# YannDubs/disentangling-vae

Hardware: AMD Instinct MI355X
Metric: images/sec (whole node) at 64x64x3, btcvae loss (higher is better)
Workload: dtype f32; 1 GPU; btcvae_celeba (BASELINE.json configs[3]): Burgess VAE 64x64x3, btcvae loss, z=10, tensor handed to _train_iteration B=1024 global (1024 per GPU), Adam lr 0.0005, n_data=202599, fwd+loss+bwd+Adam; batch_per_gpu=1024, global_batch=1024, parallelism=dp1

## Files before the change

disentangling-vae_amd/csrc/conv_up_thin_mm.hip:

```cpp
#include "recon_epilogue.h"

namespace dvae {

#define UTM_ROWS 12
#define UTM_COLS 34
#define UTM_TILE (UTM_ROWS * UTM_COLS * 32)
#define UTM_BR 11
#define UTM_NPOS (UTM_BR * 33)
#define UTM_OR 22
#define UTM_STAGE (3 * UTM_OR * 64)

__device__ __forceinline__ float sigmoid_hw_mm(float v) { return sigmoid_aten(v); }

#ifndef UTM_VARIANT
#define UTM_VARIANT 13
#endif
#ifndef UTM_ABL
#define UTM_ABL 0
#endif
__device__ __forceinline__ void utm_barrier() {
  if (UTM_VARIANT & 4) { wait_lgkmcnt0(); barrier_nofence(); }
  else __syncthreads();
}

template <bool FUSE, int DIST, typename TT>
__global__ __launch_bounds__(512, 4) void k_up_thin_mm(const float* __restrict__ small, const float* __restrict__ wimg,
                                                       const float* __restrict__ bias, float* __restrict__ out, int N,
                                                       int n_units, const TT* __restrict__ target, float* __restrict__ g,
                                                       const float* __restrict__ coef, float* __restrict__ partials) {
  extern __shared__ __attribute__((aligned(16))) float smem[];
  float* tin = smem;
  float* stage = smem + UTM_TILE;
  float* redl = stage + UTM_STAGE;
  float* wl = redl + 8;
  const int tid = threadIdx.x, lane = tid & 63;
  const int wv = __builtin_amdgcn_readfirstlane(tid >> 6);
  const int j = lane & 15, kg = lane >> 4;
  const float gs = FUSE ? coef[DVAE_C_INV_B] : 0.f;
  float lsum = 0.f;

  for (int e = tid; e < UTM_TILE / 4; e += 512) reinterpret_cast<f32x4*>(tin)[e] = f32x4{0.f, 0.f, 0.f, 0.f};

  for (int e = tid; e < 32 * 64 / 4; e += 512) reinterpret_cast<f32x4*>(wl)[e] = reinterpret_cast<const f32x4*>(wimg)[e];
  const float bv = (kg < 3 && bias) ? bias[kg] : 0.f;

  int xb[3], soff[3];
  int key0[3];
  bool x0ok[3], x1ok[3];
#pragma unroll
  for (int s = 0; s < 3; ++s) {
    const int pos0 = 16 * (3 * wv + s) + j;
    const bool pvalid = pos0 < UTM_NPOS;
    const int pos = pvalid ? pos0 : UTM_NPOS - 1;
    const int rq = pos / 33, cq = pos - 33 * rq;
    xb[s] = (rq * UTM_COLS + cq) * 32;
    key0[s] = cq & 7;
    soff[s] = (kg * UTM_OR + 2 * rq) * 64 + 2 * cq - 1;
    x0ok[s] = pvalid && kg < 3 && cq > 0;
    x1ok[s] = pvalid && kg < 3 && cq < 32;
  }
  const bool tile3 = 16 * (3 * wv + 2) < UTM_NPOS;
  const int within = tid & 255, rhalf = tid >> 8;
  const int pgo = rhalf * 1024 + within * 4;
  const int ci_ld = (within >> 3) + 1;
  const int plo = (rhalf * UTM_COLS + ci_ld) * 32 + (((within & 7) ^ (ci_ld & 7)) << 2);
  int bso[3], bgo[3], brow[3];
#pragma unroll
  for (int k = 0; k < 3; ++k) {
    const int e = tid + 512 * k;
    const int c = e / (UTM_OR * 16), rem = e - c * (UTM_OR * 16), r = rem >> 4, x4 = rem & 15;
    brow[k] = e < 3 * UTM_OR * 16 ? r : -1000;
    bso[k] = (c * UTM_OR + r) * 64 + 4 * x4;
    bgo[k] = (c * 64 + r) * 64 + 4 * x4;
  }
  __syncthreads();

  f32x4 pf[6];
  auto load_tile = [&](int unit) {
    const int n = unit / 3, u3 = unit - 3 * n;
    const int sy0 = UTM_BR * u3 - 1;
    const float* base = small + ((long)n * 32 + sy0) * 1024 + pgo;
#pragma unroll
    for (int k = 0; k < 6; ++k) {
      const int sy = sy0 + 2 * k + rhalf;
      pf[k] = f32x4{0.f, 0.f, 0.f, 0.f};
      if (sy >= 0 && sy < 32 && !((UTM_ABL & 16) && N > 0)) pf[k] = *reinterpret_cast<const f32x4*>(base + 2048 * k);
    }
  };
  if ((int)blockIdx.x < n_units) load_tile(blockIdx.x);
  for (int unit = blockIdx.x; unit < n_units; unit += gridDim.x) {
    const int n = unit / 3, u3 = unit - 3 * n;
    const int Y0 = UTM_OR * u3 - 1;
    const long img0 = ((long)n * 3 * 64 + Y0) * 64;
    f32x4 tg[3];
    uchar4 tg8[3];
    auto load_targets_k = [&](int k) {
      const int Y = Y0 + brow[k];
      tg[k] = f32x4{0.f, 0.f, 0.f, 0.f};
      tg8[k] = make_uchar4(0, 0, 0, 0);
      if (Y >= 0 && Y < 64) {
        if constexpr (sizeof(TT) == 4) tg[k] = *reinterpret_cast<const f32x4*>(target + img0 + bgo[k]);
        else tg8[k] = *reinterpret_cast<const uchar4*>(target + img0 + bgo[k]);
      }
    };
    auto load_targets = [&]() {
#pragma unroll
      for (int k = 0; k < 3; ++k) {
        const int Y = Y0 + brow[k];
        tg[k] = f32x4{0.f, 0.f, 0.f, 0.f};
        tg8[k] = make_uchar4(0, 0, 0, 0);
        if (Y >= 0 && Y < 64 && !((UTM_ABL & 4) && N > 0)) {
          if constexpr (sizeof(TT) == 4) tg[k] = *reinterpret_cast<const f32x4*>(target + img0 + bgo[k]);
          else tg8[k] = *reinterpret_cast<const uchar4*>(target + img0 + bgo[k]);
        }
      }
    };
#pragma unroll
    for (int k = 0; k < 6; ++k) *reinterpret_cast<f32x4*>(tin + plo + 2 * UTM_COLS * 32 * k) = pf[k];
    if ((UTM_VARIANT & 1) && unit + (int)gridDim.x < n_units) load_tile(unit + gridDim.x);
    if (FUSE && (UTM_VARIANT & 2)) load_targets();
    if (FUSE && (UTM_VARIANT & 16)) load_targets_k(0);
    utm_barrier();
    f32x4 acc[3];
#pragma unroll
    for (int s = 0; s < 3; ++s) acc[s] = f32x4{0.f, 0.f, 0.f, 0.f};
#pragma unroll
    for (int tap = 0; tap < 4; ++tap) {
      const int a = tap >> 1, b = tap & 1;
      f32x4 x[3][2];
      float wr[8];
#pragma unroll
      for (int i = 0; i < 8; ++i) wr[i] = wl[(tap * 8 + i) * 64 + lane];
#pragma unroll
      for (int s = 0; s < 3; ++s) {
        if (s == 2 && !tile3) continue;
        const int key = (key0[s] + b) & 7;
        const float* px = tin + xb[s] + (a * UTM_COLS + b) * 32;
        x[s][0] = *reinterpret_cast<const f32x4*>(px + (((2 * kg) ^ key) << 2));
        x[s][1] = *reinterpret_cast<const f32x4*>(px + (((2 * kg + 1) ^ key) << 2));
      }
#pragma unroll
      for (int i = 0; i < 8; ++i) {
#pragma unroll
        for (int s = 0; s < 3; ++s) {
          if (s == 2 && !tile3) continue;
          if (!((UTM_ABL & 1) && N > 0)) acc[s] = __builtin_amdgcn_mfma_f32_16x16x4f32(wr[i], x[s][i >> 2][i & 3], acc[s], 0, 0, 0);
        }
      }
    }
    if (FUSE && (UTM_VARIANT & 8)) load_targets();
    if (FUSE && (UTM_VARIANT & 16)) { load_targets_k(1); load_targets_k(2); }
#pragma unroll
    for (int s = 0; s < 3; ++s) {
      if (s == 2 && !tile3) continue;
      float* sp = stage + soff[s];
      if (x0ok[s]) { sp[0] = acc[s][0] + bv; sp[64] = acc[s][2] + bv; }
      if (x1ok[s]) { sp[1] = acc[s][1] + bv; sp[65] = acc[s][3] + bv; }
    }
    utm_barrier();
    if (!(UTM_VARIANT & 1) && unit + (int)gridDim.x < n_units) load_tile(unit + gridDim.x);
    if (FUSE && !(UTM_VARIANT & (2 | 8 | 16))) load_targets();
    if (FUSE && sizeof(TT) != 4) {
#pragma unroll
      for (int k = 0; k < 3; ++k) tg[k] = f32x4{to_unit(tg8[k].x), to_unit(tg8[k].y), to_unit(tg8[k].z), to_unit(tg8[k].w)};
    }
#pragma unroll
    for (int k = 0; k < 3; ++k) {
      const int Y = Y0 + brow[k];
      if (Y < 0 || Y >= 64) continue;
      f32x4 v = *reinterpret_cast<const f32x4*>(stage + bso[k]);
      f32x4 gl = {0.f, 0.f, 0.f, 0.f};
#pragma unroll
      for (int q = 0; q < 4; ++q) {
        if ((UTM_ABL & 2) && N > 0) {
          gl[q] = v[q] + tg[k][q];
        } else if (FUSE && DIST == DVAE_REC_BERNOULLI) {
          float y, glq;
          lsum += sigmoid_bce_logit(v[q], tg[k][q], &y, &glq);
          v[q] = y;
          gl[q] = gs * glq;
        } else {
          const float y = sigmoid_hw_mm(v[q]);
          v[q] = y;
          if (FUSE) {
            float glq, gr;
            lsum += recon_elem(y, tg[k][q], DIST, &glq, &gr);
            gl[q] = gs * glq;
          }
        }
      }
      if ((UTM_ABL & 8) && N > 0) { lsum += v[0] + v[1] + v[2] + v[3] + gl[0] + gl[1] + gl[2] + gl[3]; continue; }
      *reinterpret_cast<f32x4*>(out + img0 + bgo[k]) = v;
      if (FUSE) *reinterpret_cast<f32x4*>(g + img0 + bgo[k]) = gl;
    }
  }
  if (FUSE) {
    const float v = wave_sum(lsum);
    __syncthreads();
    if (lane == 0) redl[wv] = v;
    __syncthreads();
    if (tid == 0) {
      float s = 0.f;
#pragma unroll
      for (int w = 0; w < 8; ++w) s += redl[w];
      partials[blockIdx.x] = s;
    }
    for (int k = gridDim.x + blockIdx.x * 512 + tid; k < DVAE_REC_NPART; k += gridDim.x * 512) partials[k] = 0.f;
  }
}

int launch_up_thin_mm(const float* small, const float* wimg, const float* bias, const void* target, int target_u8, float* out,
                      float* g, int dist, const float* coef, float* partials, int N, int act, hipStream_t s) {
  static const bool off = env_off("DVAE_UP_THIN_MM");
  static const int min_n = env_int("DVAE_UP_THIN_MM_MIN_N", 1);
  if (off || N < min_n || act != DVAE_ACT_SIGMOID) return 1;
  if ((((uintptr_t)small | (uintptr_t)out | (uintptr_t)g) & 15) != 0 || ((uintptr_t)target & (target_u8 ? 3 : 15)) != 0) return 1;
  const int n_units = 3 * N;
  static const int cap = env_int("DVAE_UP_THIN_MM_GRID", 512);
  const int grid = n_units < cap ? n_units : cap;
  constexpr size_t lds = (size_t)(UTM_TILE + UTM_STAGE + 8 + 32 * 64) * sizeof(float);
#define UTM_GO(FUSE_, DIST_, TT_)                                                                                         \
  do {                                                                                                                    \
    static DeviceOnce attr;                                                                                               \
    if (attr.first())                                                                                                     \
      (void)hipFuncSetAttribute((const void*)k_up_thin_mm<FUSE_, DIST_, TT_>, hipFuncAttributeMaxDynamicSharedMemorySize, (int)lds); \
    hipLaunchKernelGGL((k_up_thin_mm<FUSE_, DIST_, TT_>), dim3(grid), dim3(512), lds, s, small, wimg, bias, out, N, n_units,      \
                       (const TT_*)target, g, coef, partials);                                                           \
  } while (0)
  if (!target) UTM_GO(false, 0, float);
  else if (target_u8) {
    if (dist == DVAE_REC_BERNOULLI) UTM_GO(true, DVAE_REC_BERNOULLI, uint8_t);
    else if (dist == DVAE_REC_GAUSSIAN) UTM_GO(true, DVAE_REC_GAUSSIAN, uint8_t);
    else UTM_GO(true, DVAE_REC_LAPLACE, uint8_t);
  } else {
    if (dist == DVAE_REC_BERNOULLI) UTM_GO(true, DVAE_REC_BERNOULLI, float);
    else if (dist == DVAE_REC_GAUSSIAN) UTM_GO(true, DVAE_REC_GAUSSIAN, float);
    else UTM_GO(true, DVAE_REC_LAPLACE, float);
  }
#undef UTM_GO
  DVAE_CHECK_LAUNCH();
  return 0;
}

}
```

Measured before the change: 991,200 images/s.

## Stream input tiles into LDS via direct global-to-LDS DMA from dedicated waves

Replaces the register-staged prefetch of the input tile (global load into registers, then LDS store) with direct global-to-LDS DMA transfers issued by the last UTM_NDW waves. The next tile is issued after the epilogue barrier and awaited with vmcnt-based waits before the compute barrier. Boundary rows are now zeroed explicitly instead of loading zeros. The third target/epilogue slot is restricted to wave 0, and the variant default changes to match the new schedule. This cuts VGPR pressure and LDS write instructions, but depends on correct vmcnt accounting and explicit zeroing of halo rows.

```diff
diff --git a/disentangling-vae_amd/csrc/conv_up_thin_mm.hip b/disentangling-vae_amd/csrc/conv_up_thin_mm.hip
--- a/disentangling-vae_amd/csrc/conv_up_thin_mm.hip
+++ b/disentangling-vae_amd/csrc/conv_up_thin_mm.hip
@@ -13,11 +13,15 @@
 __device__ __forceinline__ float sigmoid_hw_mm(float v) { return sigmoid_aten(v); }
 
 #ifndef UTM_VARIANT
-#define UTM_VARIANT 13
+#define UTM_VARIANT 12
 #endif
 #ifndef UTM_ABL
 #define UTM_ABL 0
 #endif
+#ifndef UTM_NDW
+#define UTM_NDW 2
+#endif
+static_assert(UTM_NDW == 1 || UTM_NDW == 2 || UTM_NDW == 4, "a wave's transfers stay inside one tile row; wave 0 never issues");
 __device__ __forceinline__ void utm_barrier() {
   if (UTM_VARIANT & 4) { wait_lgkmcnt0(); barrier_nofence(); }
   else __syncthreads();
@@ -42,10 +46,10 @@
   for (int e = tid; e < UTM_TILE / 4; e += 512) reinterpret_cast<f32x4*>(tin)[e] = f32x4{0.f, 0.f, 0.f, 0.f};
 
   for (int e = tid; e < 32 * 64 / 4; e += 512) reinterpret_cast<f32x4*>(wl)[e] = reinterpret_cast<const f32x4*>(wimg)[e];
-  const float bv = (kg < 3 && bias) ? bias[kg] : 0.f;
-
-  int xb[3], soff[3];
-  int key0[3];
+  float bv = (kg < 3 && bias) ? bias[kg] : 0.f;
+  asm volatile("" : "+v"(bv));
+
+  int xb[3], soff[3], key0[3];
   bool x0ok[3], x1ok[3];
 #pragma unroll
   for (int s = 0; s < 3; ++s) {
@@ -60,10 +64,9 @@
     x1ok[s] = pvalid && kg < 3 && cq < 32;
   }
   const bool tile3 = 16 * (3 * wv + 2) < UTM_NPOS;
-  const int within = tid & 255, rhalf = tid >> 8;
-  const int pgo = rhalf * 1024 + within * 4;
-  const int ci_ld = (within >> 3) + 1;
-  const int plo = (rhalf * UTM_COLS + ci_ld) * 32 + (((within & 7) ^ (ci_ld & 7)) << 2);
+  const bool dmaw = wv >= 8 - UTM_NDW, k2on = wv == 0;
+  const unsigned dvoff = (unsigned)(((lane >> 3) << 7) + (((lane & 7) ^ (((lane >> 3) + 1) & 7)) << 4));
+  const unsigned lds_tin = (unsigned)(unsigned long long)(__attribute__((address_space(3))) void*)tin;
   int bso[3], bgo[3], brow[3];
 #pragma unroll
   for (int k = 0; k < 3; ++k) {
@@ -75,30 +78,28 @@
   }
   __syncthreads();
 
-  f32x4 pf[6];
-  auto load_tile = [&](int unit) {
+  constexpr int UTM_NST = (UTM_ABL & 8) ? 0 : (FUSE ? 4 : 2);
+  constexpr int UTM_NTG = !FUSE ? 0 : (UTM_VARIANT & 2) ? ((UTM_ABL & 4) ? 0 : 2) : (UTM_VARIANT & 16) ? 1 : 0;
+  auto issue_tile = [&](int unit) {
     const int n = unit / 3, u3 = unit - 3 * n;
-    const int sy0 = UTM_BR * u3 - 1;
-    const float* base = small + ((long)n * 32 + sy0) * 1024 + pgo;
-#pragma unroll
-    for (int k = 0; k < 6; ++k) {
-      const int sy = sy0 + 2 * k + rhalf;
-      pf[k] = f32x4{0.f, 0.f, 0.f, 0.f};
-      if (sy >= 0 && sy < 32 && !((UTM_ABL & 16) && N > 0)) pf[k] = *reinterpret_cast<const f32x4*>(base + 2048 * k);
+    const float* row0 = small + ((long)n * 32 + UTM_BR * u3) * 1024 + (wv - (8 - UTM_NDW)) * 256;
+#pragma unroll
+    for (int k = 0; k < 4 * UTM_ROWS / UTM_NDW; ++k) {
+      const int ri = (UTM_NDW * k) >> 2, t = (UTM_NDW * k) & 3;
+      if ((ri == 0 && u3 == 0) || (ri == UTM_ROWS - 1 && u3 == 2) || ((UTM_ABL & 16) && N > 0)) continue;
+      const unsigned dst = lds_tin + (unsigned)((ri * UTM_COLS + 8 * t + 1) * 128) + (unsigned)(wv - (8 - UTM_NDW)) * 1024u;
+      lds_dma16_masked(row0 + (ri - 1) * 1024 + t * 256, dvoff, __builtin_amdgcn_readfirstlane(dst), ~0ull);
     }
   };
-  if ((int)blockIdx.x < n_units) load_tile(blockIdx.x);
+  if (dmaw) issue_tile(blockIdx.x);
   for (int unit = blockIdx.x; unit < n_units; unit += gridDim.x) {
-    const int n = unit / 3, u3 = unit - 3 * n;
-    const int Y0 = UTM_OR * u3 - 1;
+    const int n = unit / 3, u3 = unit - 3 * n, Y0 = UTM_OR * u3 - 1;
     const long img0 = ((long)n * 3 * 64 + Y0) * 64;
-    f32x4 tg[3];
-    uchar4 tg8[3];
+    f32x4 tg[3]; uchar4 tg8[3];
     auto load_targets_k = [&](int k) {
       const int Y = Y0 + brow[k];
-      tg[k] = f32x4{0.f, 0.f, 0.f, 0.f};
-      tg8[k] = make_uchar4(0, 0, 0, 0);
-      if (Y >= 0 && Y < 64) {
+      tg[k] = f32x4{0.f, 0.f, 0.f, 0.f}, tg8[k] = make_uchar4(0, 0, 0, 0);
+      if (Y >= 0 && Y < 64 && (k < 2 || k2on)) {
         if constexpr (sizeof(TT) == 4) tg[k] = *reinterpret_cast<const f32x4*>(target + img0 + bgo[k]);
         else tg8[k] = *reinterpret_cast<const uchar4*>(target + img0 + bgo[k]);
       }
@@ -107,19 +108,17 @@
 #pragma unroll
       for (int k = 0; k < 3; ++k) {
         const int Y = Y0 + brow[k];
-        tg[k] = f32x4{0.f, 0.f, 0.f, 0.f};
-        tg8[k] = make_uchar4(0, 0, 0, 0);
-        if (Y >= 0 && Y < 64 && !((UTM_ABL & 4) && N > 0)) {
+        tg[k] = f32x4{0.f, 0.f, 0.f, 0.f}, tg8[k] = make_uchar4(0, 0, 0, 0);
+        if (Y >= 0 && Y < 64 && (k < 2 || k2on) && !((UTM_ABL & 4) && N > 0)) {
           if constexpr (sizeof(TT) == 4) tg[k] = *reinterpret_cast<const f32x4*>(target + img0 + bgo[k]);
           else tg8[k] = *reinterpret_cast<const uchar4*>(target + img0 + bgo[k]);
         }
       }
     };
-#pragma unroll
-    for (int k = 0; k < 6; ++k) *reinterpret_cast<f32x4*>(tin + plo + 2 * UTM_COLS * 32 * k) = pf[k];
-    if ((UTM_VARIANT & 1) && unit + (int)gridDim.x < n_units) load_tile(unit + gridDim.x);
+    if (u3 != 1 && tid < 256) reinterpret_cast<f32x4*>(tin + ((u3 ? UTM_ROWS - 1 : 0) * UTM_COLS + 1) * 32)[tid] = f32x4{0.f, 0.f, 0.f, 0.f};
     if (FUSE && (UTM_VARIANT & 2)) load_targets();
     if (FUSE && (UTM_VARIANT & 16)) load_targets_k(0);
+    if (dmaw) { if (unit == (int)blockIdx.x) wait_vmcnt<UTM_NTG>(); else wait_vmcnt<UTM_NTG + UTM_NST>(); }
     utm_barrier();
     f32x4 acc[3];
 #pragma unroll
@@ -158,16 +157,17 @@
       if (x1ok[s]) { sp[1] = acc[s][1] + bv; sp[65] = acc[s][3] + bv; }
     }
     utm_barrier();
-    if (!(UTM_VARIANT & 1) && unit + (int)gridDim.x < n_units) load_tile(unit + gridDim.x);
     if (FUSE && !(UTM_VARIANT & (2 | 8 | 16))) load_targets();
     if (FUSE && sizeof(TT) != 4) {
 #pragma unroll
       for (int k = 0; k < 3; ++k) tg[k] = f32x4{to_unit(tg8[k].x), to_unit(tg8[k].y), to_unit(tg8[k].z), to_unit(tg8[k].w)};
     }
+    if (FUSE) asm volatile("" : "+v"(tg[0]), "+v"(tg[1]), "+v"(tg[2]));
+    if (dmaw && unit + (int)gridDim.x < n_units) issue_tile(unit + gridDim.x);
 #pragma unroll
     for (int k = 0; k < 3; ++k) {
       const int Y = Y0 + brow[k];
-      if (Y < 0 || Y >= 64) continue;
+      if (Y < 0 || Y >= 64 || (k == 2 && !k2on)) continue;
       f32x4 v = *reinterpret_cast<const f32x4*>(stage + bso[k]);
       f32x4 gl = {0.f, 0.f, 0.f, 0.f};
 #pragma unroll
```

New measurement: 988,800 images/s. Within noise of the previous version (-0.2%).
